# zhuker/lamejs

Hardware: NVIDIA H100
Metric: encoded audio seconds/sec (44.1kHz stereo 128kbps CBR) (higher is better)
Workload: dtype f64

## Files before the change

lamejs_b200/csrc/k_filterbank.cuh:

```cuda
#ifndef MP3B200_K_FILTERBANK_CUH
#define MP3B200_K_FILTERBANK_CUH
#include "mp3_device.cuh"

#define FB_G 8
#define FB_SPAN (576 * FB_G + 1055)
#define FB_PCM_WORDS (FB_SPAN + (FB_SPAN >> 5) + 2)
#define FB_SLAB_STRIDE 33
#define FB_THREADS 192

__constant__ double c_enwindow[285];
__constant__ double c_mdct_win[4 * 36];
__constant__ int c_sb_order[32];

#define EW(i) c_enwindow[(i)]
#define MWIN(t, i) c_mdct_win[(t) * 36 + (i)]
#define WS(i) c_mdct_win[2 * 36 + (i)]
#define SQRT2_D 1.41421356237309504880

__device__ __forceinline__ int fb_pad(int i) { return i + (i >> 5); }

__device__ __forceinline__ void window_subband_dev(const double* __restrict__ x, int p0, f32s* a) {
#define X1(o) (x[fb_pad(x1p + (o))])
#define X2(o) (x[fb_pad(x2p + (o))])
  int x1p = p0, x2p = p0 + 238 - 14 - 286;
// ... 299 lines not shown
  for (int w = tid; w < scount * 18; w += FB_THREADS) {
    const int s = w / 18, j = w - s * 18;
    f32s a[32];
    window_subband_dev(pcm, 576 * s + 286 + 32 * j, a);
    f32s* row = slab + (s * 18 + j) * FB_SLAB_STRIDE;
#pragma unroll
    for (int p = 0; p < 32; p++) {
      double v = a[p];
      if ((j & 1) && (p & 1)) v = v * -1;
      const float amp = s_amp[p];
      f32s r; r = v;
      if ((double)amp < 1.0 && !((double)amp < 1e-12)) r *= (double)amp;
      row[p] = r;
    }
  }
  __syncthreads();
  float* const dst = slab_out + (((size_t)sd.unit_base + z + u0 + 1) * nch + ch) * 576;
  for (int w = tid; w < scount * 576; w += FB_THREADS) {
    const int s = w / 576, r = w - s * 576;
    dst[(size_t)s * nch * 576 + r] = slab[(s * 18 + (r >> 5)) * FB_SLAB_STRIDE + (r & 31)].v;
  }
}

__global__ void __launch_bounds__(FB_G * 32)
k_mdct(const Mp3Tables* __restrict__ T, const StreamDesc* __restrict__ streams, const float* __restrict__ slab_in,
       const signed char* __restrict__ blocktype, float* __restrict__ xr_out) {
  const int z = blockIdx.z;
  const StreamDesc& sd = streams[z];
  const int ch = blockIdx.y;
  const int ngr = sd.nframes * T->mode_gr;
  const int g0 = blockIdx.x * FB_G;
  if (g0 >= ngr) return;
  const int gcount = min(FB_G, ngr - g0);
  const int nch = T->nch;
  __shared__ f32s xr[FB_G * 576];
  __shared__ float s_amp[32];
  __shared__ int s_bt[FB_G];
  const int tid = threadIdx.x;
  if (tid < 32) s_amp[c_sb_order[tid]] = T->amp_filter[tid];
  if (tid < gcount) s_bt[tid] = blocktype[(size_t)(sd.unit_base + g0 + tid) * 2 + ch];
  __syncthreads();

  {
    const int g = tid >> 5, band = tid & 31;
    if (g < gcount) {
      const int type = s_bt[g];
      const int ob = c_sb_order[band];
      f32s* o = xr + g * 576 + band * 18;
      if ((double)s_amp[ob] < 1e-12) {
#pragma unroll
        for (int k = 0; k < 18; k++) o[k] = 0.0;
      } else {
        const float* p0 = slab_in + (((size_t)sd.unit_base + z + g0 + g) * nch + ch) * 576 + ob;
        const float* p1 = p0 + (size_t)nch * 576;
        float b0[18], b1[18];
#pragma unroll
        for (int k = 0; k < 18; k++) { b0[k] = __ldg(p0 + 32 * k); b1[k] = __ldg(p1 + 32 * k); }
#define B0(k) ((double)b0[(k)])
#define B1(k) ((double)b1[(k)])
        if (type == BT_SHORT) {
          f32s io[18];
#pragma unroll
          for (int k = -3; k < 0; k++) {
            const double wv = WS(k + 3);
            io[k * 3 + 9] = B0(9 + k) * wv - B0(8 - k);
            io[k * 3 + 18] = B0(14 - k) * wv + B0(15 + k);
            io[k * 3 + 10] = B0(15 + k) * wv - B0(14 - k);
            io[k * 3 + 19] = B1(2 - k) * wv + B1(3 + k);
            io[k * 3 + 11] = B1(3 + k) * wv - B1(2 - k);
            io[k * 3 + 20] = B1(8 - k) * wv + B1(9 + k);
          }
          mdct_short_dev(io);
#pragma unroll
          for (int k = 0; k < 18; k++) o[k] = (double)io[k];
        } else {
          f32s work[18];
#pragma unroll
          for (int k = -9; k < 0; k++) {
            double a, b;
            a = MWIN(type, k + 27) * B1(k + 9) + MWIN(type, k + 36) * B1(8 - k);
            b = MWIN(type, k + 9) * B0(k + 9) - MWIN(type, k + 18) * B0(8 - k);
            work[k + 9] = a - b * WS(3 + k + 9);
            work[k + 18] = a * WS(3 + k + 9) + b;
          }
          mdct_long_dev(o, work);
        }
#undef B0
#undef B1
      }
    }
  }
  __syncthreads();

  for (int w = tid; w < gcount * 31 * 8; w += FB_G * 32) {
    const int g = w / 248, r = w - g * 248;
    const int band = 1 + (r >> 3), k = r & 7;
    if (s_bt[g] == BT_SHORT) continue;
    f32s* e = xr + g * 576 + band * 18;
    const double lo_v = e[-1 - k], hi_v = e[k];
    const double bu = hi_v * WS(20 + k) + lo_v * WS(28 + k);
    const double bd = hi_v * WS(28 + k) - lo_v * WS(20 + k);
    e[-1 - k] = bu;
    e[k] = bd;
  }
  __syncthreads();
  for (int w = tid; w < gcount * 576; w += FB_G * 32) {
    const int g = w / 576, i = w - g * 576;
    xr_out[((size_t)(sd.unit_base + g0 + g) * nch + ch) * 576 + i] = xr[w].v;
  }
}

#endif
```

lamejs_b200/csrc/k_psy.cuh:

```cuda
#ifndef MP3B200_K_PSY_CUH
#define MP3B200_K_PSY_CUH
#include "mp3_device.cuh"
#include "mp3_tables.h"

#ifndef PSY_THREADS
#define PSY_THREADS 128
#endif
#define MASK_THREADS 128

struct PsyUnit {
  float eb_l[MP3_CBANDS];
  float peaks[9];
  float loudness;
  unsigned char mask_idx[MP3_CBANDS];
  unsigned char attack[4];
  unsigned char pad_;
};
struct PsyShort {
  double ecb_s[3][MP3_CBANDS];
  float eb_s[3][MP3_CBANDS];
};
struct PsyRatioDev { float en_l[22], thm_l[22], en_s[13][3], thm_s[13][3]; };

__constant__ unsigned char c_fft_rv[128];
// ... 683 lines not shown
      return m1 * ((c_table1[i] - f) * r + f);
    }
    if (i > 13) return m1;
    return m1 * c_table3[i];
  }
  return m1 * c_table1[i];
}

__global__ void __launch_bounds__(MASK_THREADS)
k_psy_masking(const Mp3Tables* __restrict__ T, const StreamDesc* __restrict__ streams, const PsyUnit* __restrict__ psy,
              const PsyShort* __restrict__ psy_s, const signed char* __restrict__ bt_prev, const signed char* __restrict__ bt_final,
              int all_short, const double* __restrict__ ath_psy, PsyRatioDev* __restrict__ ratio) {
  const int z = blockIdx.z;
  const StreamDesc& sd = streams[z];
  const int u = (int)blockIdx.x - 1;
  if (u >= T->mode_gr * sd.nframes) return;
  const int nch = T->nch;
  const long long c = (long long)T->mode_gr * sd.frame0 + u;
  const int tid = threadIdx.x, ch = tid >> 6, b = tid & 63;
  PsyRatioDev* out = ratio + psy_row(sd, z, u) * nch;
  if (u < 0) {
    if (c < 0) {
      const float big = (float)1e20;
      for (int i = tid; i < nch * 122; i += MASK_THREADS) (&out[0].en_l[0])[i] = big;
    }
    else if (sd.halo_in) {
      for (int i = tid; i < nch * 122; i += MASK_THREADS) (&out[0].en_l[0])[i] = sd.halo_in[i];
    }
    return;
  }
  __shared__ f32s s_thr[2][MP3_CBANDS + 2], s_eb[2][MP3_CBANDS + 2];
  __shared__ f32s s_thr_s[2][3][MP3_CBANDS + 2];
  __shared__ PsyRatioDev s_out[2];
  const int npl = T->npart_l, nps = T->npart_s;
  const PsyUnit* pu = (ch < nch) ? psy + psy_row(sd, z, u) * nch + ch : nullptr;
  const PsyShort* ps = (ch < nch) ? psy_s + psy_row(sd, z, u) * nch + ch : nullptr;
  const PsyShort* pp = (ch < nch) ? psy_s + psy_row(sd, z, u - 1) * nch + ch : nullptr;
  const bool short_read = psy_short_read(T, sd, bt_final, u, all_short);
  const double ath_adjust = ath_psy[sd.frame_base + u / T->mode_gr];

  if (ch < nch) {
    if (b < npl) {
      int kk = T->s3lo_l[b];
      int k = T->s3off_l[b];
      double eb2 = (double)pu->eb_l[kk] * c_tab[pu->mask_idx[kk]];
      double ecb = (double)T->s3_ll[k++] * eb2;
      while (++kk <= T->s3hi_l[b]) {
        eb2 = (double)pu->eb_l[kk] * c_tab[pu->mask_idx[kk]];
        ecb = mask_add_dev(ecb, (double)T->s3_ll[k++] * eb2, kk, kk - b, T, ath_adjust);
      }
// ... 59 lines not shown
      if (bd >= 0) {
        const double w_curr = (double)T->bo_s_weight[sbi];
        en[sbi][sblock] += w_curr * (double)ps->eb_s[sblock][bd];
        thm[sbi][sblock] += w_curr * (double)s_thr_s[ch][sblock][bd];
      }
    }
    const double e3 = (double)pu->peaks[sblock * 3 + 0], e4 = (double)pu->peaks[sblock * 3 + 1], e5 = (double)pu->peaks[sblock * 3 + 2];
    double t = (double)thm[sbi][sblock];
    t *= 0.8;
    const double enn2 = e3 + e4 + e5;
    if (e5 * 6 < enn2) { t *= 0.5; if (e4 * 6 < enn2) t *= 0.5; }
    thm[sbi][sblock] = t;
  }
  __syncthreads();
  if (nch == 2 && T->interch_ratio > 0.0 && tid < (short_read ? 22 + 39 : 22)) {
    const double r = T->interch_ratio;
    f32s* t0 = reinterpret_cast<f32s*>(tid < 22 ? &s_out[0].thm_l[tid] : &s_out[0].thm_s[0][0] + (tid - 22));
    f32s* t1 = reinterpret_cast<f32s*>(tid < 22 ? &s_out[1].thm_l[tid] : &s_out[1].thm_s[0][0] + (tid - 22));
    const double l = (double)*t0, rr = (double)*t1;
    *t0 += rr * r;
    *t1 += l * r;
  }
  __syncthreads();
  for (int i = tid; i < nch * 122; i += MASK_THREADS)
    if (short_read || i % 122 < 44) (&out[0].en_l[0])[i] = (&s_out[0].en_l[0])[i];
  if (sd.halo_out && u == T->mode_gr * sd.nframes - 1)
    for (int i = tid; i < nch * 122; i += MASK_THREADS) sd.halo_out[i] = (&s_out[0].en_l[0])[i];
}

#endif
```

lamejs_b200/csrc/k_quant.cuh:

```cuda
#ifndef MP3B200_K_QUANT_CUH
#define MP3B200_K_QUANT_CUH
#include <stddef.h>
#include "mp3_device.cuh"
#include "mp3_tables.h"
#include "k_psy.cuh"

#define Q_LARGE_BITS 100000
#define Q_IXMAX 8206
#define Q_FULL 0xffffffffu

struct GranuleInfoDev {
  int global_gain, part2_3_length, part2_length, big_values, count1, scalefac_compress;
  int table_select[3], region0_count, region1_count, preflag, scalefac_scale, count1table_select, block_type;
  int subblock_gain[4];
  int count1bits, sfbmax, sfbdivide, sfb_lmax, psymax, psy_lmax, sfb_smin, max_nonzero_coeff;
  int scalefac[MP3_SFBMAX];
  int slen[4];
  int part_row;
  int pad_;
  double xrpow_max;
};
struct QuantFrameState {
  int stream, rel_frame;
  int in_old[2], in_step[2];
// ... 829 lines not shown
    } else {
      if (++age > search_limit && best.over_count == 0) break;
    }
    const int cont = (wk->w.global_gain + wk->w.scalefac_scale) < 255;
    __syncwarp();
    if (!cont) break;
  } while (true);
  if (!best_here) copy_ix_w(wk->ixw, wk->ixg);
}

__device__ __noinline__ double ath_adjust_dev(double a, double x, double athFloor) {
  const double o = 90.30873362, p = 94.82444863;
  double u = q_log10(x) * 10.0;
  const double v = a * a;
  double w = 0.0;
  u -= athFloor;
  if (v > 1E-20) w = 1. + q_log10(v) * (10.0 / o);
  if (w < 0) w = 0.;
  u *= w;
  u += athFloor + o - p;
  return q_pow(10., 0.1 * u);
}

__device__ __noinline__ bool gc_prepare_w(const Mp3Tables* T, GcWork* wk, const double* ath_ps, const float* __restrict__ xr_g, int block_type,
                             const PsyRatioDev* __restrict__ ratio, double ath_adjust) {
  const bool need_xmin = true;
  const int lane = LANE;
  GranuleInfoDev* gi = &wk->b;
  const bool is_short = block_type == BT_SHORT;
  if (lane == 0) {
    gi->part2_3_length = 0; gi->big_values = 0; gi->count1 = 0; gi->global_gain = 210; gi->scalefac_compress = 0;
    gi->table_select[0] = gi->table_select[1] = gi->table_select[2] = 0;
    gi->subblock_gain[0] = gi->subblock_gain[1] = gi->subblock_gain[2] = gi->subblock_gain[3] = 0;
    gi->region0_count = 0; gi->region1_count = 0; gi->preflag = 0; gi->scalefac_scale = 0; gi->count1table_select = 0;
    gi->part2_length = 0; gi->block_type = block_type; gi->count1bits = 0;
    gi->sfb_lmax = is_short ? 0 : 21; gi->sfb_smin = is_short ? 0 : 12;
    gi->psy_lmax = is_short ? 0 : 21;
    gi->psymax = is_short ? 36 : 21; gi->sfbmax = is_short ? 36 : 21; gi->sfbdivide = is_short ? 18 : 11;
    gi->max_nonzero_coeff = 575;
#pragma unroll 1
    for (int i = 0; i < MP3_SFBMAX; i++) gi->scalefac[i] = 0;
    gi->xrpow_max = 0;
  }
  const Mp3Geo* geo = &T->geo[is_short ? 1 : 0];
  if (lane == 0) wk->geo = geo;
  {
    float4 v[5];
#pragma unroll
    for (int k = 0; k < 5; k++) { const int q = lane + 32 * k; if (q < 144) v[k] = __ldg(reinterpret_cast<const float4*>(xr_g) + q); }
    if (!is_short) {
#pragma unroll
      for (int k = 0; k < 5; k++) { const int q = lane + 32 * k; if (q < 144) reinterpret_cast<float4*>(wk->xr)[q] = v[k]; }
    } else {
#pragma unroll
      for (int k = 0; k < 5; k++) {
        const int q = lane + 32 * k;
        if (q < 144) {
          const short* ro = geo->reorder + 4 * q;
          wk->xr[__ldg(ro + 0)] = v[k].x; wk->xr[__ldg(ro + 1)] = v[k].y; wk->xr[__ldg(ro + 2)] = v[k].z; wk->xr[__ldg(ro + 3)] = v[k].w;
        }
      }
    }
  }
  __syncwarp();
  if (!is_short) {
    const int lo = T->psfb21[0];
    const double lf = (double)T->longfact[21];
    int keep = lo - 1;
#pragma unroll 1
    for (int j = lo + lane; j < 576; j += 32) {
      int g = 0;
      while (g < 5 && j >= T->psfb21[g + 1]) g++;
      double ath21 = ath_ps[g];
      if (lf > 1e-12) ath21 *= lf;
      if (!(fabs((double)wk->xr[j]) < ath21)) keep = j;
    }
    keep = wmax(keep);
    __syncwarp();
#pragma unroll 1
    for (int j = keep + 1 + lane; j < 576; j += 32) wk->xr[j] = 0.0f;
  } else if (lane == 0) {
#pragma unroll 1
    for (int block = 0; block < 3; block++) {
      bool stop = false;
#pragma unroll 1
// ... 585 lines not shown

__device__ __forceinline__ int granule_budget(int nch, int mean_bits, int gr, int used0, int used1, int ch) {
  int tbits = mean_bits;
  if (gr == 1) {
    const int resv = -(used0 + (nch == 2 ? used1 : 0)) + mean_bits;
    if (resv * 10 > 0) tbits += resv;
  }
  double t = (double)tbits / nch;
  if (t > 4095) t = 4095;
  int targ = (int)t;
  const int bits = targ * nch;
  if (bits > 7680) { targ = targ * 7680; targ = (int)((double)targ / bits); }
  (void)ch;
  return targ;
}

#ifndef Q_WARPS
#define Q_WARPS 4
#endif
#ifndef Q_BLOCKS_PER_SM
#define Q_BLOCKS_PER_SM 7
#endif
#define Q_THREADS (32 * Q_WARPS)

__device__ __forceinline__ int next_task(int* counter) {
  int t = 0;
  if (LANE == 0) t = atomicAdd(counter, 1);
  return __shfl_sync(Q_FULL, t, 0);
}
template <int STRIDE = (int)sizeof(WarpShared)>
__device__ __forceinline__ WarpShared* warp_shared() {
  extern __shared__ __align__(16) unsigned char smem_raw[];
  return reinterpret_cast<WarpShared*>(smem_raw + (threadIdx.x >> 5) * STRIDE);
}
__device__ __forceinline__ void gi_init_w(GranuleInfoDev* gi, const GcPrep* __restrict__ pr) {
  __syncwarp();
  int* w = reinterpret_cast<int*>(gi);
#pragma unroll 1
  for (int i = LANE; i < (int)(sizeof(GranuleInfoDev) / 4); i += 32) w[i] = 0;
  __syncwarp();
  if (LANE == 0) {
    const int bt = pr->block_type;
    const bool is_short = bt == BT_SHORT;
    gi->global_gain = 210; gi->block_type = bt;
    gi->sfb_lmax = is_short ? 0 : 21; gi->sfb_smin = is_short ? 0 : 12; gi->psy_lmax = is_short ? 0 : 21;
    gi->psymax = is_short ? 36 : 21; gi->sfbmax = is_short ? 36 : 21; gi->sfbdivide = is_short ? 18 : 11;
// ... 2 lines not shown
  __syncwarp();
}
__device__ __forceinline__ void copy_row16_w(void* dst, const void* src, int nbytes) {
  __syncwarp();
  const int n = nbytes >> 4;
  int4 v[5];
#pragma unroll
  for (int k = 0; k < 5; k++) { const int i = LANE + 32 * k; if (i < n) v[k] = reinterpret_cast<const int4*>(src)[i]; }
#pragma unroll
  for (int k = 0; k < 5; k++) { const int i = LANE + 32 * k; if (i < n) reinterpret_cast<int4*>(dst)[i] = v[k]; }
  __syncwarp();
}
struct FrameGeom { int z, f, padding, frame_bytes, mean_bits; long long kabs; };
__device__ __forceinline__ FrameGeom frame_geom(const Mp3Tables* T, const StreamDesc* streams, const QuantFrameState* q) {
  FrameGeom g;
  g.z = q->stream; g.f = q->rel_frame;
  g.kabs = (long long)streams[g.z].frame0 + g.f;
  g.padding = (int)(pad_count(g.kabs, T->frac_SpF, T->samplerate) - pad_count(g.kabs - 1, T->frac_SpF, T->samplerate));
  g.frame_bytes = T->frame_bytes_nopad + g.padding;
  g.mean_bits = (8 * g.frame_bytes - T->sideinfo_len * 8) / T->mode_gr;
  return g;
}

__global__ void __launch_bounds__(Q_THREADS, Q_BLOCKS_PER_SM)
k_q_prepare(const Mp3Tables* __restrict__ T, const StreamDesc* __restrict__ streams, const float* __restrict__ xr,
            const PsyRatioDev* __restrict__ ratio, const signed char* __restrict__ bt_final, const double* __restrict__ ath_q,
            const QuantFrameState* __restrict__ qs, float* __restrict__ xrq, float* __restrict__ xrpow_g, unsigned* __restrict__ neg_g,
            GcPrep* __restrict__ prep,
            int nframes, int* __restrict__ counter) {
  WarpShared* ws = warp_shared();
  GcWork* wk = &ws->wk;
  const int lane = LANE, nch = T->nch;
  const int G = T->mode_gr;
  const int ntasks = nframes * G * nch;
#pragma unroll 1
  for (int t = next_task(counter); t < ntasks; t = next_task(counter)) {
    const int frow = t / (G * nch), rem = t - frow * G * nch, gr = rem / nch, ch = rem - gr * nch;
    const QuantFrameState* q = qs + frow;
    const int z = q->stream, f = q->rel_frame;
    const StreamDesc& sd = streams[z];
    const double ath_adjust = ath_q[frow];
    const size_t urow = (size_t)sd.unit_base + G * f + gr, gidx = urow * nch + ch;
    const int bt = bt_final[urow * 2 + ch];
    const PsyRatioDev* rt = ratio + ((size_t)sd.unit_base + z + G * f + gr) * nch + ch;
    __syncwarp();
    if (lane < 6) ws->ath[lane] = ath_adjust_dev(ath_adjust, (double)(bt == BT_SHORT ? T->ath_psfb12[lane] : T->ath_psfb21[lane]), T->ath_floor);
    __syncwarp();
    const bool have = gc_prepare_w(T, wk, ws->ath, xr + gidx * 576, bt, rt, ath_adjust);
    copy_row16_w(xrq + gidx * 576, wk->xr, 2304);
    {
      unsigned mine = 0;
#pragma unroll 1
      for (int k = 0; k < 18; k++) { const unsigned m = __ballot_sync(Q_FULL, wk->xr[lane + 32 * k] < 0.0f); if (lane == k) mine = m; }
      if (lane < 18) neg_g[gidx * 18 + lane] = mine;
    }
    copy_row16_w(xrpow_g + gidx * 576, wk->xrpow, 2304);
    GcPrep* pr = prep + gidx;
#pragma unroll 1
    for (int i = lane; i < MP3_SFBMAX; i += 32) pr->xmin[i] = wk->xmin[i];
    if (lane == 0) { pr->have = have ? 1 : 0; pr->mnz = wk->b.max_nonzero_coeff; pr->block_type = bt; pr->xrpow_max = wk->b.xrpow_max; }
  }
}

__global__ void __launch_bounds__(Q_THREADS, Q_SLIM_BLOCKS)
k_q_search(const Mp3Tables* __restrict__ T, const StreamDesc* __restrict__ streams, QuantFrameState* __restrict__ qs,
           GranuleInfoDev* __restrict__ ginfo, short* __restrict__ l3enc, const float* __restrict__ xrpow_g,
           const GcPrep* __restrict__ prep, int gr, const int* __restrict__ list, const int* __restrict__ count_ptr, int count_direct,
           int revalidate, int* __restrict__ counter, int* __restrict__ list2, int* __restrict__ count2,
           int* __restrict__ list3, int* __restrict__ count3) {
  WarpShared* ws = warp_shared<Q_STRIDE_NOXR>();
  GcWork* wk = &ws->wk;
// ... 260 lines not shown

__global__ void k_qstate_commit(StreamDesc* __restrict__ streams, int nstreams, const QuantFrameState* __restrict__ qs) {
  const int z = blockIdx.x * blockDim.x + threadIdx.x;
  if (z >= nstreams) return;
  StreamDesc& sd = streams[z];
  if (sd.nframes <= 0) return;
  const QuantFrameState* q = qs + sd.frame_base + sd.nframes - 1;
#pragma unroll 1
  for (int c = 0; c < 2; c++) { sd.old_value[c] = q->out_old[c]; sd.current_step[c] = q->out_step[c]; }
}

__global__ void k_qstate_loop_cond(cudaGraphConditionalHandle loop, int* __restrict__ count, int* __restrict__ st, int max_passes) {
  const int n = *count;
  int passes = st[2];
  bool more = n != 0;
  if (more) passes++;
  if (passes > max_passes) { st[1] = 1; *count = 0; more = false; }
  st[2] = passes;
  if (passes > st[0]) st[0] = passes;
  cudaGraphSetConditional(loop, more ? 1u : 0u);
}

struct QuantBuffers {
  const float* xr; const PsyRatioDev* ratio; const signed char* bt; const double* ath_q;
  QuantFrameState* qs; GranuleInfoDev* ginfo; short* l3enc; float* xrq; float* xrpow; unsigned* neg; GcPrep* prep;
  int* over_budget;
  int* list; int* counter;
};
#define Q_NCOUNTERS 256
#define Q_REPAIR_BLOCKS 16
enum { QE_START, QE_PREP, QE_S0, QE_O0, QE_F0, QE_S1, QE_MID, QE_O1, QE_F1, QE_PK, QE_COUNT };

struct QuantLoop {
  cudaStream_t capture = nullptr;
  int* st = nullptr;
  cudaGraphExec_t exec = nullptr;
};

static int quant_run(const Mp3Tables* dT, const Mp3Tables& hT, StreamDesc* d_streams, int S, int nstreams_with_frames, int max_frames, long long F,
                     const QuantBuffers& B, cudaStream_t st_main, cudaStream_t st_repair, cudaEvent_t ev_fork, cudaEvent_t ev_join,
                     cudaEvent_t ev_pass1, cudaEvent_t* evq, int* evq_pred, int* passes_out, std::atomic<long long>* launches,
                     QuantLoop* dloop = nullptr) {
  cudaStream_t st = st_main;
  static std::mutex attr_mu;
  static bool attr_done[64] = {};
  int dev = 0, sms = 132;
  cudaGetDevice(&dev);
// ... 12 lines not shown
  }
  if (F <= 0) { *passes_out = 0; return 0; }
  const int nch = hT.nch;
  int next_counter = Q_NCOUNTERS;
  auto fresh_counter = [&]() -> int* {
    if (next_counter >= Q_NCOUNTERS) { cudaMemsetAsync(B.counter + 3, 0, sizeof(int) * (Q_NCOUNTERS - 3), st); next_counter = 3; }
    return B.counter + next_counter++;
  };
  auto grid_for = [&](long long tasks, int per_sm) -> int {
    long long g = (tasks + Q_WARPS - 1) / Q_WARPS, cap = (long long)sms * per_sm;
    if (g > cap) g = cap;
    return (int)(g < 1 ? 1 : g);
  };
  {
    dim3 g((max_frames + 127) / 128, S);
    k_qstate_init<<<g, 128, 0, st>>>(d_streams, S, B.qs);
    (*launches)++;
  }
  for (int i = 0; i < QE_COUNT; i++) evq_pred[i] = -1;
  int last_slot = -1;
  auto mark = [&](int slot) { cudaEventRecord(evq[slot], st); evq_pred[slot] = last_slot; last_slot = slot; };
  int* const prep_counter = fresh_counter();
  mark(QE_START);
  k_q_prepare<<<grid_for(F * hT.mode_gr * nch, Q_BLOCKS_PER_SM), Q_THREADS, smem, st>>>(dT, d_streams, B.xr, B.ratio, B.bt, B.ath_q, B.qs, B.xrq, B.xrpow, B.neg,
                                                                              B.prep, (int)F, prep_counter);
  mark(QE_PREP);
  (*launches)++;
  int* const list1 = B.list;
  int* const list2 = B.list + (F + 1);
  int* const list3 = B.list + 2 * (F + 1);
  auto search = [&](int gr, const int* list, const int* cptr, long long count, int reval) {
    k_q_search<<<grid_for(count * nch, Q_SLIM_BLOCKS), Q_THREADS, smem_slim, st>>>(dT, d_streams, B.qs, B.ginfo, B.l3enc, B.xrpow, B.prep, gr, list, cptr, (int)count,
                                                                             reval, fresh_counter(), list2, B.counter + 1, list3, B.counter + 2);
    (*launches)++;
  };
  int reserve_blocks = 0;
  auto finish = [&](int gr, const int* list, const int* cptr, long long count, int reval) {
    k_q_finish<<<max(1, grid_for(count * nch, Q_SLIM_BLOCKS) - reserve_blocks), Q_THREADS, smem_slim, st>>>(dT, d_streams, B.qs, B.ginfo, B.l3enc, gr, list, cptr, (int)count, reval, fresh_counter());
    (*launches)++;
  };
  auto outer = [&](int gr, const int* list, const int* cptr, long long count, int reval) {
    k_q_outer<<<max(1, grid_for(count * nch, Q_BLOCKS_PER_SM) - reserve_blocks), Q_THREADS, smem, st>>>(dT, d_streams, B.qs, B.ginfo, B.l3enc, B.xrq, B.xrpow, B.prep, gr, list, cptr, (int)count,
                                                                            reval, fresh_counter());
    (*launches)++;
  };
  auto outer_finish = [&](int gr, long long count, int reval, int slot_o, int slot_f) {
    outer(gr, nullptr, nullptr, count, reval); mark(slot_o);
    finish(gr, nullptr, nullptr, count, reval); mark(slot_f);
  };
  auto pack = [&](const int* list, const int* cptr, long long count, int reval) {
// ... 117 lines not shown
```

lamejs_b200/csrc/mp3_encoder.cu:

```cuda
#include <cuda_runtime.h>
#include <math.h>
#include <stdio.h>
#include <algorithm>
#include <array>
#include <stdlib.h>
#include <string.h>
#include <atomic>
#include <map>
#include <mutex>
#include <string>
#include <tuple>
#include <vector>

#include "../../include/mp3b200.h"
#include "mp3_config.h"
#include "mp3_device.cuh"
#include "mp3_tables.h"
#include "k_filterbank.cuh"
#include "k_psy.cuh"
#include "k_quant.cuh"
#include "k_tag.cuh"
#include "k_resample.cuh"
#include "k_replaygain.cuh"
#include "k_stage.cuh"
// ... 164 lines not shown
  Buf<int> short_count;
  Buf<ScanIn> scan_in;
  Buf<PsyRatioDev> ratio;
  Buf<double> ath_psy;
  Buf<double> ath_q;
  Buf<QuantFrameState> qstate;
  Buf<GranuleInfoDev> ginfo;
  Buf<short> l3enc;
  Buf<float> xrq;
  Buf<float> xrpow;
  Buf<unsigned> neg;
  Buf<GcPrep> prep;
  Buf<int> dirty;
  Buf<int> counter;
  Buf<ScanChunk> scan;
  Buf<ResampleDesc> rs_desc;
  Buf<float> rs_y;
  Buf<StageDesc> st_desc;
  Buf<float> st_y;
  Buf<int> refusals;
  int fit(int S, int nch, long long U, long long F) {
    const size_t gc = (size_t)U * nch, rows = (size_t)(U + S) * nch, f = (size_t)F + 1;
    const bool failed = streams.fit(S) || bt_final.fit((size_t)U * 2 + 16) || bt_prev.fit((size_t)U * 2 + 16) ||
                        xr.fit(gc * 576) || slab.fit(rows * 576) || psy.fit(rows) || psy_s.fit(rows) || short_list.fit(rows) ||
                        short_count.fit(2) || scan_in.fit(rows) || ratio.fit(rows) ||
                        ath_psy.fit(f) || ath_q.fit(f) || qstate.fit(f) || ginfo.fit(gc) || l3enc.fit(gc * 576) ||
                        xrq.fit(gc * 576) || xrpow.fit(gc * 576) || neg.fit(gc * 18) || prep.fit(gc) || dirty.fit(3 * f) ||
                        counter.fit(Q_NCOUNTERS) || scan.fit((size_t)(F / SCAN_FRAMES + S + 1));
    return failed ? MP3B200_ERR_CUDA : 0;
  }
  size_t generation() const {
    return streams.cap + qstate.cap + ginfo.cap + l3enc.cap + xrq.cap + xrpow.cap + neg.cap + prep.cap + dirty.cap + counter.cap +
           refusals.cap;
  }
  void release() {
    streams.release(); bt_final.release(); bt_prev.release(); xr.release(); slab.release(); psy.release(); psy_s.release(); short_list.release();
    short_count.release(); scan_in.release();
    ratio.release(); ath_psy.release(); ath_q.release(); qstate.release(); ginfo.release(); l3enc.release(); xrq.release();
    xrpow.release(); neg.release(); prep.release(); dirty.release(); counter.release(); scan.release();
    rs_desc.release(); rs_y.release(); st_desc.release(); st_y.release(); refusals.release();
  }
};

struct PinnedArena { uint8_t* p = nullptr; size_t cap = 0, used = 0; };

enum { MP3_MAX_PCM_CHUNKS = 8 };
enum { MP3_MAX_LAUNCH_STREAMS = 65535 };
// ... 130 lines not shown

struct Timings { float psy = 0, scan = 0, mask = 0, fb = 0, q1 = 0, qn = 0, total = 0; int passes = 0;
                 float q_prepare = 0, q_search = 0, q_outer = 0, q_finish = 0, q_pack = 0, q_mid = 0; };

struct PcmArrival { int chunks = 1; cudaEvent_t* ready = nullptr; };

int refusal_error(int refused, int over_budget, int fault) {
  if (refused) { g_err = "non-finite input sample (or one beyond 2^40 once scaled)"; return MP3B200_ERR_CONFIG; }
  if (over_budget) { g_err = "frame over its bit budget (input too loud to encode)"; return MP3B200_ERR_CONFIG; }
  if (fault == RG_FAULT) { g_err = "ReplayGain repair did not converge"; return MP3B200_ERR_CUDA; }
  if (fault) { g_err = "quantizer stage failed: the fixed-point loop did not converge"; return MP3B200_ERR_CUDA; }
  return 0;
}

int check_refusals(ThreadCtx& c) {
  int r[2] = {0, 0};
  CK(cudaMemcpyAsync(r, c.ws.refusals.p, sizeof r, cudaMemcpyDeviceToHost, c.st));
  CK(cudaStreamSynchronize(c.st));
  return refusal_error(r[0], r[1], 0);
}

struct LaunchOpts {
  const int32_t* force_bt = nullptr;
  bool stop_after_mdct = false;
  bool all_short = false;
  const PcmArrival* arrival = nullptr;
  float* timings_ms = nullptr;
  bool sync = true;
  struct RgJob* rg = nullptr;
  bool f32_in = false;
  struct LoopGraphs* loops = nullptr;
  const struct HandleCarry* carry = nullptr;
  int* rg_loop = nullptr;
  bool analyse_only = false;
};

struct HandleCarry { HandleRecord* const* recs; float* halo_scratch; };

enum { MP3_RG_GRAPHS = 32 };
struct LoopGraphs {
  cudaStream_t capture = nullptr;
  size_t generation = 0, rg_generation = 0;
  long long instantiated = 0;
  unsigned long long rg_tick = 0;
  std::map<std::tuple<const Config*, int, long long, int>, cudaGraphExec_t> exec;
  struct RgGraph { cudaGraphExec_t exec = nullptr; unsigned long long used = 0; };
  std::map<std::tuple<const Config*, bool, int, int, long long, const int*>, RgGraph> rg_exec;
// ... 198 lines not shown
    std::vector<signed char> bt((size_t)units * 2, 0);
    for (long long u = 0; u < units; u++)
      for (int c = 0; c < nch; c++) bt[u * 2 + c] = (signed char)o.force_bt[u * nch + c];
    CK(cudaMemcpyAsync(ws.bt_final.p, bt.data(), bt.size(), cudaMemcpyHostToDevice, st));
    CK(cudaStreamSynchronize(st));
  }
  {
    CK(cudaMemsetAsync(ws.short_count.p, 0, 2 * sizeof(int), st));
    dim3 grid((cfg->host.mode_gr * max_frames + 1 + 127) / 128, S);
    k_psy_short_list<<<grid, 128, 0, st>>>(tab, ws.streams.p, ws.bt_final.p, o.all_short ? 1 : 0, ws.short_list.p, ws.short_count.p);
    DBG("k_psy_short_list");
    int sms = 132;
    CK(cudaDeviceGetAttribute(&sms, cudaDevAttrMultiProcessorCount, c.device));
    const long long tasks = ((long long)cfg->host.mode_gr * total_frames + S) * nch;
    const int blocks = (int)std::min<long long>(std::max<long long>(tasks, 1), (long long)sms * PSY_SHORT_BLOCKS);
    if (f32_pcm) k_psy_short<true><<<blocks, PSY_THREADS, 0, st>>>(tab, ws.streams.p, ws.psy_s.p, ws.short_list.p, ws.short_count.p);
    else k_psy_short<false><<<blocks, PSY_THREADS, 0, st>>>(tab, ws.streams.p, ws.psy_s.p, ws.short_list.p, ws.short_count.p);
    g_launches += 2;
    DBG("k_psy_short");
    if (psy_launch >= 0 && (rc = psy_record_short(c, h_streams, nch, cfg->host.mode_gr, psy_launch, k2_launches))) return rc;
  }
  {
    dim3 grid(cfg->host.mode_gr * max_frames + 1, 1, S);
    k_psy_masking<<<grid, MASK_THREADS, 0, st>>>(tab, ws.streams.p, ws.psy.p, ws.psy_s.p, ws.bt_prev.p, ws.bt_final.p,
                                                 o.all_short ? 1 : 0, ws.ath_psy.p, ws.ratio.p);
    g_launches++;
    DBG("k_psy_masking");
  }
  CK(cudaEventRecord(ev[3], st));
  {
    dim3 grid((cfg->host.mode_gr * max_frames + FB_G - 1) / FB_G, nch, S);
    k_mdct<<<grid, FB_G * 32, 0, st>>>(tab, ws.streams.p, ws.slab.p, ws.bt_final.p, ws.xr.p);
    g_launches++;
    DBG("k_mdct");
  }
  CK(cudaEventRecord(ev[4], st));
  int passes = 0;
  if (!o.stop_after_mdct) {
    QuantBuffers qb;
    qb.xr = ws.xr.p; qb.ratio = ws.ratio.p; qb.bt = ws.bt_final.p; qb.ath_q = ws.ath_q.p; qb.qs = ws.qstate.p; qb.ginfo = ws.ginfo.p;
    qb.l3enc = ws.l3enc.p; qb.xrq = ws.xrq.p; qb.xrpow = ws.xrpow.p; qb.neg = ws.neg.p; qb.prep = ws.prep.p; qb.list = ws.dirty.p; qb.counter = ws.counter.p;
    qb.over_budget = ws.refusals.p + 1;
    QuantLoop dloop;
    cudaGraphExec_t* cached = nullptr;
    if (o.loops) {
      LoopGraphs& lg = *o.loops;
      if (lg.generation != ws.generation()) { lg.clear(); lg.generation = ws.generation(); }
      cached = &lg.exec[std::make_tuple((const Config*)cfg, S, total_frames, max_frames)];
      dloop.capture = lg.capture; dloop.st = ws.refusals.p + 2; dloop.exec = *cached;
    }
    rc = quant_run(tab, cfg->host, ws.streams.p, S, streams_with_frames, max_frames, total_frames, qb, st, c.aux_st, c.ev_fork, c.ev_join, ev[5], c.evq, c.evq_pred, &passes, &g_launches,
                   o.loops ? &dloop : nullptr);
    if (cached) {
      if (!*cached && dloop.exec) o.loops->instantiated++;
      *cached = dloop.exec;
      if (!dloop.exec) o.loops->exec.erase(std::make_tuple((const Config*)cfg, S, total_frames, max_frames));
    }
    if (rc) { g_err = "quantizer stage failed: " + std::string(cudaGetErrorString(cudaGetLastError())); return rc; }
  } else {
    CK(cudaEventRecord(ev[5], st));
  }
  CK(cudaEventRecord(ev[6], st));
  if (!o.sync) return 0;
  CK(cudaStreamSynchronize(st));
  CK(cudaGetLastError());
  if (tm) {
    cudaEventElapsedTime(&tm->psy, ev[0], ev[1]);
    cudaEventElapsedTime(&tm->scan, ev[1], ev[2]);
    cudaEventElapsedTime(&tm->mask, ev[2], ev[3]);
    cudaEventElapsedTime(&tm->fb, ev[3], ev[4]);
    cudaEventElapsedTime(&tm->q1, ev[4], ev[5]);
    cudaEventElapsedTime(&tm->qn, ev[5], ev[6]);
    cudaEventElapsedTime(&tm->total, ev[0], ev[6]);
    tm->passes = passes;
    if (!o.stop_after_mdct && passes > 0) {
      auto span = [&](int slot) { float v = 0; const int p = c.evq_pred[slot]; if (p >= 0) cudaEventElapsedTime(&v, c.evq[p], c.evq[slot]); return v; };
      tm->q_prepare = span(QE_PREP);
      tm->q_search = span(QE_S0) + span(QE_S1);
      tm->q_outer = span(QE_O0) + span(QE_O1);
      tm->q_finish = span(QE_F0) + span(QE_F1);
      tm->q_pack = span(QE_PK);
      tm->q_mid = span(QE_MID);
    }
  }
  return 0;
}

void init_stream_state(StreamDesc& sd) {
  sd.ath_adjust = 0.01; sd.ath_adjust_limit = 1.0;
  sd.blocktype_old[0] = sd.blocktype_old[1] = BT_NORM;
  sd.last_attacks[0] = sd.last_attacks[1] = 0;
  sd.old_value[0] = sd.old_value[1] = 180;
  sd.current_step[0] = sd.current_step[1] = 4;
}

long long hist_base_at(int mode_gr, long long frame) {
  const long long b = 576LL * mode_gr * frame - 1104;
  return b > 0 ? b : 0;
// ... 371 lines not shown
    }
    if (o.rg) {
      rc = rg_queue(c, cfg, group, *o.rg, arrival, rows);
      if (rc) return rc;
    }
    Timings tm;
    rc = o.analyse_only ? 0 : run_pipeline(c, cfg, group, n, o, arrival, rows, &tm);
    if (rc) return rc;
    if (o.rg) {
      rc = o.loops ? rg_finish_queued(c, cfg, *o.rg, *o.loops, o.rg_loop ? o.rg_loop : c.ws.refusals.p + 5, c.ws.refusals.p + 3)
                   : rg_finish(c, cfg, *o.rg);
      if (rc) return rc;
    }
    arrival = nullptr;
    float rs_ms = 0.0f;
    if (resampled && o.timings_ms && o.sync) CK(cudaEventElapsedTime(&rs_ms, c.ev_rs[0], c.ev_rs[1]));
    if (o.timings_ms) {
      const float t[16] = {tm.psy, tm.scan, tm.mask, tm.fb, tm.q1, tm.qn, tm.total, 0.0f,
                           tm.q_prepare, tm.q_search, tm.q_outer, tm.q_finish, tm.q_pack, tm.q_mid, rs_ms, 0.0f};
      for (int i = 0; i < 16; i++) o.timings_ms[i] += t[i];
      if ((float)tm.passes > o.timings_ms[7]) o.timings_ms[7] = (float)tm.passes;
    }
  }
  return o.sync && (o.f32_in || !o.stop_after_mdct) ? check_refusals(c) : 0;
}

}

extern "C" {

const char* mp3b200_last_error(void) { return g_err.c_str(); }
#ifdef Q_STATS
int mp3b200_debug_qstats(unsigned long long* out16, int reset) {
  if (cudaMemcpyFromSymbol(out16, g_qstats, sizeof(unsigned long long) * 16) != cudaSuccess) return MP3B200_ERR_CUDA;
  if (reset) { unsigned long long z[16] = {0}; cudaMemcpyToSymbol(g_qstats, z, sizeof z); }
  return 0;
}
#endif
int64_t mp3b200_launch_count(void) { return g_launches; }
int mp3b200_debug_psy_capture(int on) {
  std::lock_guard<std::mutex> lk(g_psy_mu);
  if (on) { g_psy_rec.clear(); g_psy_launch = 0; }
  g_psy_capture.store(on ? 1 : 0);
  return 0;
}
int64_t mp3b200_debug_psy_take(void* buf, int64_t cap) {
  std::lock_guard<std::mutex> lk(g_psy_mu);
// ... 513 lines not shown
  uint8_t* bytes_out = tp->bytes_out;
  const int64_t bytes_cap = tp->bytes_cap;
  Config* cfg;
  int rc = get_config(channels, tp->samplerate, tp->kbps, tp->flags & ~MP3B200_DEBUG_SKIP_SHORT, &cfg);
  if (rc || (rc = check_input(cfg, 1, &left, &right, &nsamples))) return rc;
  const int nch = cfg->host.nch;
  const int G = cfg->host.mode_gr;
  const StreamPlan pl = stream_plan(cfg, 1, &nsamples, false, nullptr);
  const long long F = pl.frames[0], U = G * F, nbytes = pl.audio[0];
  std::vector<int64_t> pcm_off;
  T* d_pcm = nullptr;
  PcmArrival arr;
  if ((rc = upload_host_rows(cfg, 1, &left, &right, &nsamples, pcm_off, d_pcm, arr)) || (rc = t_ctx.out.fit((size_t)nbytes + 8))) return rc;
  uint8_t* d_out = t_ctx.out.p;
  const int64_t zero = 0;
  std::vector<StreamDesc> sds = whole_streams(cfg, pl, 1, d_pcm, pcm_off.data(), &nsamples, d_out, &zero);
  const bool want_gi = ginfo || tp->scalefac || tp->subblock_gain;
  const bool want_prep = tp->xmin || tp->max_nonzero_coeff || tp->xrpow_max;
  const bool want_q = tp->scfsi || tp->old_value || tp->cur_step;
  LaunchOpts opts;
  opts.f32_in = std::is_same_v<T, float>;
  opts.force_bt = force_blocktype;
  opts.all_short = !(tp->flags & MP3B200_DEBUG_SKIP_SHORT);
  opts.stop_after_mdct = !(l3_enc || bytes_out || want_gi || want_prep || want_q);
  opts.arrival = &arr;
  rc = launch_streams(t_ctx, cfg, sds, opts);
  auto fetch = [](void* dst, const void* src, size_t bytes) {
    const cudaError_t e = cudaMemcpyAsync(dst, src, bytes, cudaMemcpyDeviceToHost, t_ctx.st);
    return e != cudaSuccess ? e : cudaStreamSynchronize(t_ctx.st);
  };
  const Workspace& ws = t_ctx.ws;
  if (rc == 0) {
    if (xr) CK(fetch(xr, ws.xr.p, sizeof(float) * (size_t)U * nch * 576));
    if (blocktype) {
      std::vector<signed char> bt((size_t)U * 2);
      CK(fetch(bt.data(), ws.bt_final.p, bt.size()));
      for (long long u = 0; u < U; u++) for (int c = 0; c < nch; c++) blocktype[u * nch + c] = bt[u * 2 + c];
    }
    if (en_l || thm_l || en_s || thm_s) {
      std::vector<PsyRatioDev> r((size_t)(U + 1) * nch);
      CK(fetch(r.data(), ws.ratio.p, sizeof(PsyRatioDev) * r.size()));
      for (long long u = 0; u < U; u++) for (int c = 0; c < nch; c++) {
        const PsyRatioDev& q = r[(size_t)u * nch + c];
        if (en_l) memcpy(en_l + (u * nch + c) * 22, q.en_l, sizeof q.en_l);
        if (thm_l) memcpy(thm_l + (u * nch + c) * 22, q.thm_l, sizeof q.thm_l);
        if (en_s) memcpy(en_s + (u * nch + c) * 39, q.en_s, sizeof q.en_s);
        if (thm_s) memcpy(thm_s + (u * nch + c) * 39, q.thm_s, sizeof q.thm_s);
// ... 250 lines not shown
```

Measured before the change: 61490.

## Fuse MDCT into quantizer prepare kernel and size masking block by channels

Removes the standalone k_mdct kernel and computes each granule's MDCT, including alias reduction, inside k_q_prepare. One warp does this per granule and writes straight into the working buffer, so the xr round-trip through global memory and one kernel launch go away. The xr buffer is kept only as an optional debug tap, and short-block reordering now happens in shared memory. k_psy_masking is also launched with 64*nch threads, and its strided loops use blockDim, so stereo runs at the same 128 threads. The cost is that MDCT now runs warp-serial per granule inside a kernel tuned for quantizer occupancy, which may add pressure on registers or time.

```diff
diff --git a/lamejs_b200/csrc/k_filterbank.cuh b/lamejs_b200/csrc/k_filterbank.cuh
--- a/lamejs_b200/csrc/k_filterbank.cuh
+++ b/lamejs_b200/csrc/k_filterbank.cuh
@@ -345,92 +345,69 @@
   }
 }
 
-__global__ void __launch_bounds__(FB_G * 32)
-k_mdct(const Mp3Tables* __restrict__ T, const StreamDesc* __restrict__ streams, const float* __restrict__ slab_in,
-       const signed char* __restrict__ blocktype, float* __restrict__ xr_out) {
-  const int z = blockIdx.z;
-  const StreamDesc& sd = streams[z];
-  const int ch = blockIdx.y;
-  const int ngr = sd.nframes * T->mode_gr;
-  const int g0 = blockIdx.x * FB_G;
-  if (g0 >= ngr) return;
-  const int gcount = min(FB_G, ngr - g0);
-  const int nch = T->nch;
-  __shared__ f32s xr[FB_G * 576];
-  __shared__ float s_amp[32];
-  __shared__ int s_bt[FB_G];
-  const int tid = threadIdx.x;
-  if (tid < 32) s_amp[c_sb_order[tid]] = T->amp_filter[tid];
-  if (tid < gcount) s_bt[tid] = blocktype[(size_t)(sd.unit_base + g0 + tid) * 2 + ch];
-  __syncthreads();
-
-  {
-    const int g = tid >> 5, band = tid & 31;
-    if (g < gcount) {
-      const int type = s_bt[g];
-      const int ob = c_sb_order[band];
-      f32s* o = xr + g * 576 + band * 18;
-      if ((double)s_amp[ob] < 1e-12) {
-#pragma unroll
-        for (int k = 0; k < 18; k++) o[k] = 0.0;
-      } else {
-        const float* p0 = slab_in + (((size_t)sd.unit_base + z + g0 + g) * nch + ch) * 576 + ob;
-        const float* p1 = p0 + (size_t)nch * 576;
-        float b0[18], b1[18];
-#pragma unroll
-        for (int k = 0; k < 18; k++) { b0[k] = __ldg(p0 + 32 * k); b1[k] = __ldg(p1 + 32 * k); }
+__device__ __forceinline__ void mdct_granule_w(const Mp3Tables* __restrict__ T, const float* __restrict__ slab_prev, int nch, int type,
+                                               f32s* xr) {
+  const int band = threadIdx.x & 31;
+  {
+    const int ob = c_sb_order[band];
+    f32s* o = xr + band * 18;
+    if ((double)T->amp_filter[band] < 1e-12) {
+#pragma unroll
+      for (int k = 0; k < 18; k++) o[k] = 0.0;
+    } else {
+      const float* p0 = slab_prev + ob;
+      const float* p1 = p0 + (size_t)nch * 576;
+      float b0[18], b1[18];
+#pragma unroll
+      for (int k = 0; k < 18; k++) { b0[k] = __ldg(p0 + 32 * k); b1[k] = __ldg(p1 + 32 * k); }
 #define B0(k) ((double)b0[(k)])
 #define B1(k) ((double)b1[(k)])
-        if (type == BT_SHORT) {
-          f32s io[18];
-#pragma unroll
-          for (int k = -3; k < 0; k++) {
-            const double wv = WS(k + 3);
-            io[k * 3 + 9] = B0(9 + k) * wv - B0(8 - k);
-            io[k * 3 + 18] = B0(14 - k) * wv + B0(15 + k);
-            io[k * 3 + 10] = B0(15 + k) * wv - B0(14 - k);
-            io[k * 3 + 19] = B1(2 - k) * wv + B1(3 + k);
-            io[k * 3 + 11] = B1(3 + k) * wv - B1(2 - k);
-            io[k * 3 + 20] = B1(8 - k) * wv + B1(9 + k);
-          }
-          mdct_short_dev(io);
-#pragma unroll
-          for (int k = 0; k < 18; k++) o[k] = (double)io[k];
-        } else {
-          f32s work[18];
-#pragma unroll
-          for (int k = -9; k < 0; k++) {
-            double a, b;
-            a = MWIN(type, k + 27) * B1(k + 9) + MWIN(type, k + 36) * B1(8 - k);
-            b = MWIN(type, k + 9) * B0(k + 9) - MWIN(type, k + 18) * B0(8 - k);
-            work[k + 9] = a - b * WS(3 + k + 9);
-            work[k + 18] = a * WS(3 + k + 9) + b;
-          }
-          mdct_long_dev(o, work);
+      if (type == BT_SHORT) {
+        f32s io[18];
+#pragma unroll
+        for (int k = -3; k < 0; k++) {
+          const double wv = WS(k + 3);
+          io[k * 3 + 9] = B0(9 + k) * wv - B0(8 - k);
+          io[k * 3 + 18] = B0(14 - k) * wv + B0(15 + k);
+          io[k * 3 + 10] = B0(15 + k) * wv - B0(14 - k);
+          io[k * 3 + 19] = B1(2 - k) * wv + B1(3 + k);
+          io[k * 3 + 11] = B1(3 + k) * wv - B1(2 - k);
+          io[k * 3 + 20] = B1(8 - k) * wv + B1(9 + k);
         }
+        mdct_short_dev(io);
+#pragma unroll
+        for (int k = 0; k < 18; k++) o[k] = (double)io[k];
+      } else {
+        f32s work[18];
+#pragma unroll
+        for (int k = -9; k < 0; k++) {
+          double a, b;
+          a = MWIN(type, k + 27) * B1(k + 9) + MWIN(type, k + 36) * B1(8 - k);
+          b = MWIN(type, k + 9) * B0(k + 9) - MWIN(type, k + 18) * B0(8 - k);
+          work[k + 9] = a - b * WS(3 + k + 9);
+          work[k + 18] = a * WS(3 + k + 9) + b;
+        }
+        mdct_long_dev(o, work);
+      }
 #undef B0
 #undef B1
-      }
     }
   }
-  __syncthreads();
-
-  for (int w = tid; w < gcount * 31 * 8; w += FB_G * 32) {
-    const int g = w / 248, r = w - g * 248;
-    const int band = 1 + (r >> 3), k = r & 7;
-    if (s_bt[g] == BT_SHORT) continue;
-    f32s* e = xr + g * 576 + band * 18;
-    const double lo_v = e[-1 - k], hi_v = e[k];
-    const double bu = hi_v * WS(20 + k) + lo_v * WS(28 + k);
-    const double bd = hi_v * WS(28 + k) - lo_v * WS(20 + k);
-    e[-1 - k] = bu;
-    e[k] = bd;
-  }
-  __syncthreads();
-  for (int w = tid; w < gcount * 576; w += FB_G * 32) {
-    const int g = w / 576, i = w - g * 576;
-    xr_out[((size_t)(sd.unit_base + g0 + g) * nch + ch) * 576 + i] = xr[w].v;
-  }
+  __syncwarp();
+
+  if (type != BT_SHORT) {
+#pragma unroll 1
+    for (int r = band; r < 31 * 8; r += 32) {
+      f32s* e = xr + (1 + (r >> 3)) * 18;
+      const int k = r & 7;
+      const double lo_v = e[-1 - k], hi_v = e[k];
+      const double bu = hi_v * WS(20 + k) + lo_v * WS(28 + k);
+      const double bd = hi_v * WS(28 + k) - lo_v * WS(20 + k);
+      e[-1 - k] = bu;
+      e[k] = bd;
+    }
+  }
+  __syncwarp();
 }
 
 #endif
diff --git a/lamejs_b200/csrc/k_psy.cuh b/lamejs_b200/csrc/k_psy.cuh
--- a/lamejs_b200/csrc/k_psy.cuh
+++ b/lamejs_b200/csrc/k_psy.cuh
@@ -729,10 +729,10 @@
   if (u < 0) {
     if (c < 0) {
       const float big = (float)1e20;
-      for (int i = tid; i < nch * 122; i += MASK_THREADS) (&out[0].en_l[0])[i] = big;
+      for (int i = tid; i < nch * 122; i += (int)blockDim.x) (&out[0].en_l[0])[i] = big;
     }
     else if (sd.halo_in) {
-      for (int i = tid; i < nch * 122; i += MASK_THREADS) (&out[0].en_l[0])[i] = sd.halo_in[i];
+      for (int i = tid; i < nch * 122; i += (int)blockDim.x) (&out[0].en_l[0])[i] = sd.halo_in[i];
     }
     return;
   }
@@ -838,10 +838,10 @@
     *t1 += l * r;
   }
   __syncthreads();
-  for (int i = tid; i < nch * 122; i += MASK_THREADS)
+  for (int i = tid; i < nch * 122; i += (int)blockDim.x)
     if (short_read || i % 122 < 44) (&out[0].en_l[0])[i] = (&s_out[0].en_l[0])[i];
   if (sd.halo_out && u == T->mode_gr * sd.nframes - 1)
-    for (int i = tid; i < nch * 122; i += MASK_THREADS) sd.halo_out[i] = (&s_out[0].en_l[0])[i];
-}
-
-#endif
+    for (int i = tid; i < nch * 122; i += (int)blockDim.x) sd.halo_out[i] = (&s_out[0].en_l[0])[i];
+}
+
+#endif
diff --git a/lamejs_b200/csrc/k_quant.cuh b/lamejs_b200/csrc/k_quant.cuh
--- a/lamejs_b200/csrc/k_quant.cuh
+++ b/lamejs_b200/csrc/k_quant.cuh
@@ -875,7 +875,7 @@
   return q_pow(10., 0.1 * u);
 }
 
-__device__ __noinline__ bool gc_prepare_w(const Mp3Tables* T, GcWork* wk, const double* ath_ps, const float* __restrict__ xr_g, int block_type,
+__device__ __noinline__ bool gc_prepare_w(const Mp3Tables* T, GcWork* wk, const double* ath_ps, int block_type,
                              const PsyRatioDev* __restrict__ ratio, double ath_adjust) {
   const bool need_xmin = true;
   const int lane = LANE;
@@ -897,23 +897,13 @@
   }
   const Mp3Geo* geo = &T->geo[is_short ? 1 : 0];
   if (lane == 0) wk->geo = geo;
-  {
-    float4 v[5];
-#pragma unroll
-    for (int k = 0; k < 5; k++) { const int q = lane + 32 * k; if (q < 144) v[k] = __ldg(reinterpret_cast<const float4*>(xr_g) + q); }
-    if (!is_short) {
-#pragma unroll
-      for (int k = 0; k < 5; k++) { const int q = lane + 32 * k; if (q < 144) reinterpret_cast<float4*>(wk->xr)[q] = v[k]; }
-    } else {
-#pragma unroll
-      for (int k = 0; k < 5; k++) {
-        const int q = lane + 32 * k;
-        if (q < 144) {
-          const short* ro = geo->reorder + 4 * q;
-          wk->xr[__ldg(ro + 0)] = v[k].x; wk->xr[__ldg(ro + 1)] = v[k].y; wk->xr[__ldg(ro + 2)] = v[k].z; wk->xr[__ldg(ro + 3)] = v[k].w;
-        }
-      }
-    }
+  if (is_short) {
+    __syncwarp();
+#pragma unroll 1
+    for (int i = lane; i < 576; i += 32) wk->xrpow[i] = wk->xr[i];
+    __syncwarp();
+#pragma unroll 1
+    for (int i = lane; i < 576; i += 32) wk->xr[__ldg(geo->reorder + i)] = wk->xrpow[i];
   }
   __syncwarp();
   if (!is_short) {
@@ -1545,6 +1535,9 @@
 #define Q_BLOCKS_PER_SM 7
 #endif
 #define Q_THREADS (32 * Q_WARPS)
+#ifndef Q_PREP_BLOCKS
+#define Q_PREP_BLOCKS Q_BLOCKS_PER_SM
+#endif
 
 __device__ __forceinline__ int next_task(int* counter) {
   int t = 0;
@@ -1593,9 +1586,9 @@
   return g;
 }
 
-__global__ void __launch_bounds__(Q_THREADS, Q_BLOCKS_PER_SM)
-k_q_prepare(const Mp3Tables* __restrict__ T, const StreamDesc* __restrict__ streams, const float* __restrict__ xr,
-            const PsyRatioDev* __restrict__ ratio, const signed char* __restrict__ bt_final, const double* __restrict__ ath_q,
+__global__ void __launch_bounds__(Q_THREADS, Q_PREP_BLOCKS)
+k_q_prepare(const Mp3Tables* __restrict__ T, const StreamDesc* __restrict__ streams, const float* __restrict__ slab,
+            float* __restrict__ xr_tap, const PsyRatioDev* __restrict__ ratio, const signed char* __restrict__ bt_final, const double* __restrict__ ath_q,
             const QuantFrameState* __restrict__ qs, float* __restrict__ xrq, float* __restrict__ xrpow_g, unsigned* __restrict__ neg_g,
             GcPrep* __restrict__ prep,
             int nframes, int* __restrict__ counter) {
@@ -1615,9 +1608,11 @@
     const int bt = bt_final[urow * 2 + ch];
     const PsyRatioDev* rt = ratio + ((size_t)sd.unit_base + z + G * f + gr) * nch + ch;
     __syncwarp();
+    mdct_granule_w(T, slab + (((size_t)sd.unit_base + z + G * f + gr) * nch + ch) * 576, nch, bt, reinterpret_cast<f32s*>(wk->xr));
+    if (xr_tap) copy_row16_w(xr_tap + gidx * 576, wk->xr, 2304);
     if (lane < 6) ws->ath[lane] = ath_adjust_dev(ath_adjust, (double)(bt == BT_SHORT ? T->ath_psfb12[lane] : T->ath_psfb21[lane]), T->ath_floor);
     __syncwarp();
-    const bool have = gc_prepare_w(T, wk, ws->ath, xr + gidx * 576, bt, rt, ath_adjust);
+    const bool have = gc_prepare_w(T, wk, ws->ath, bt, rt, ath_adjust);
     copy_row16_w(xrq + gidx * 576, wk->xr, 2304);
     {
       unsigned mine = 0;
@@ -1924,7 +1919,10 @@
 }
 
 struct QuantBuffers {
-  const float* xr; const PsyRatioDev* ratio; const signed char* bt; const double* ath_q;
+  const float* slab;
+  float* xr_tap;
+  bool prepare_only;
+  const PsyRatioDev* ratio; const signed char* bt; const double* ath_q;
   QuantFrameState* qs; GranuleInfoDev* ginfo; short* l3enc; float* xrq; float* xrpow; unsigned* neg; GcPrep* prep;
   int* over_budget;
   int* list; int* counter;
@@ -1983,10 +1981,11 @@
   auto mark = [&](int slot) { cudaEventRecord(evq[slot], st); evq_pred[slot] = last_slot; last_slot = slot; };
   int* const prep_counter = fresh_counter();
   mark(QE_START);
-  k_q_prepare<<<grid_for(F * hT.mode_gr * nch, Q_BLOCKS_PER_SM), Q_THREADS, smem, st>>>(dT, d_streams, B.xr, B.ratio, B.bt, B.ath_q, B.qs, B.xrq, B.xrpow, B.neg,
+  k_q_prepare<<<grid_for(F * hT.mode_gr * nch, Q_PREP_BLOCKS), Q_THREADS, smem, st>>>(dT, d_streams, B.slab, B.xr_tap, B.ratio, B.bt, B.ath_q, B.qs, B.xrq, B.xrpow, B.neg,
                                                                               B.prep, (int)F, prep_counter);
   mark(QE_PREP);
   (*launches)++;
+  if (B.prepare_only) { *passes_out = 0; return 0; }
   int* const list1 = B.list;
   int* const list2 = B.list + (F + 1);
   int* const list3 = B.list + 2 * (F + 1);
diff --git a/lamejs_b200/csrc/mp3_encoder.cu b/lamejs_b200/csrc/mp3_encoder.cu
--- a/lamejs_b200/csrc/mp3_encoder.cu
+++ b/lamejs_b200/csrc/mp3_encoder.cu
@@ -210,7 +210,7 @@
   int fit(int S, int nch, long long U, long long F) {
     const size_t gc = (size_t)U * nch, rows = (size_t)(U + S) * nch, f = (size_t)F + 1;
     const bool failed = streams.fit(S) || bt_final.fit((size_t)U * 2 + 16) || bt_prev.fit((size_t)U * 2 + 16) ||
-                        xr.fit(gc * 576) || slab.fit(rows * 576) || psy.fit(rows) || psy_s.fit(rows) || short_list.fit(rows) ||
+                        slab.fit(rows * 576) || psy.fit(rows) || psy_s.fit(rows) || short_list.fit(rows) ||
                         short_count.fit(2) || scan_in.fit(rows) || ratio.fit(rows) ||
                         ath_psy.fit(f) || ath_q.fit(f) || qstate.fit(f) || ginfo.fit(gc) || l3enc.fit(gc * 576) ||
                         xrq.fit(gc * 576) || xrpow.fit(gc * 576) || neg.fit(gc * 18) || prep.fit(gc) || dirty.fit(3 * f) ||
@@ -387,7 +387,8 @@
 
 struct LaunchOpts {
   const int32_t* force_bt = nullptr;
-  bool stop_after_mdct = false;
+  bool stop_after_prepare = false;
+  bool taps = false;
   bool all_short = false;
   const PcmArrival* arrival = nullptr;
   float* timings_ms = nullptr;
@@ -632,23 +633,19 @@
   }
   {
     dim3 grid(cfg->host.mode_gr * max_frames + 1, 1, S);
-    k_psy_masking<<<grid, MASK_THREADS, 0, st>>>(tab, ws.streams.p, ws.psy.p, ws.psy_s.p, ws.bt_prev.p, ws.bt_final.p,
-                                                 o.all_short ? 1 : 0, ws.ath_psy.p, ws.ratio.p);
+    k_psy_masking<<<grid, 64 * nch, 0, st>>>(tab, ws.streams.p, ws.psy.p, ws.psy_s.p, ws.bt_prev.p, ws.bt_final.p,
+                                             o.all_short ? 1 : 0, ws.ath_psy.p, ws.ratio.p);
     g_launches++;
     DBG("k_psy_masking");
   }
   CK(cudaEventRecord(ev[3], st));
-  {
-    dim3 grid((cfg->host.mode_gr * max_frames + FB_G - 1) / FB_G, nch, S);
-    k_mdct<<<grid, FB_G * 32, 0, st>>>(tab, ws.streams.p, ws.slab.p, ws.bt_final.p, ws.xr.p);
-    g_launches++;
-    DBG("k_mdct");
-  }
   CK(cudaEventRecord(ev[4], st));
   int passes = 0;
-  if (!o.stop_after_mdct) {
+  {
+    if (o.taps && ws.xr.fit((size_t)cfg->host.mode_gr * total_frames * nch * 576)) return MP3B200_ERR_CUDA;
     QuantBuffers qb;
-    qb.xr = ws.xr.p; qb.ratio = ws.ratio.p; qb.bt = ws.bt_final.p; qb.ath_q = ws.ath_q.p; qb.qs = ws.qstate.p; qb.ginfo = ws.ginfo.p;
+    qb.slab = ws.slab.p; qb.xr_tap = o.taps ? ws.xr.p : nullptr; qb.prepare_only = o.stop_after_prepare;
+    qb.ratio = ws.ratio.p; qb.bt = ws.bt_final.p; qb.ath_q = ws.ath_q.p; qb.qs = ws.qstate.p; qb.ginfo = ws.ginfo.p;
     qb.l3enc = ws.l3enc.p; qb.xrq = ws.xrq.p; qb.xrpow = ws.xrpow.p; qb.neg = ws.neg.p; qb.prep = ws.prep.p; qb.list = ws.dirty.p; qb.counter = ws.counter.p;
     qb.over_budget = ws.refusals.p + 1;
     QuantLoop dloop;
@@ -667,8 +664,7 @@
       if (!dloop.exec) o.loops->exec.erase(std::make_tuple((const Config*)cfg, S, total_frames, max_frames));
     }
     if (rc) { g_err = "quantizer stage failed: " + std::string(cudaGetErrorString(cudaGetLastError())); return rc; }
-  } else {
-    CK(cudaEventRecord(ev[5], st));
+    if (o.stop_after_prepare) CK(cudaEventRecord(ev[5], st));
   }
   CK(cudaEventRecord(ev[6], st));
   if (!o.sync) return 0;
@@ -683,7 +679,7 @@
     cudaEventElapsedTime(&tm->qn, ev[5], ev[6]);
     cudaEventElapsedTime(&tm->total, ev[0], ev[6]);
     tm->passes = passes;
-    if (!o.stop_after_mdct && passes > 0) {
+    if (!o.stop_after_prepare && passes > 0) {
       auto span = [&](int slot) { float v = 0; const int p = c.evq_pred[slot]; if (p >= 0) cudaEventElapsedTime(&v, c.evq[p], c.evq[slot]); return v; };
       tm->q_prepare = span(QE_PREP);
       tm->q_search = span(QE_S0) + span(QE_S1);
@@ -1101,7 +1097,7 @@
       if ((float)tm.passes > o.timings_ms[7]) o.timings_ms[7] = (float)tm.passes;
     }
   }
-  return o.sync && (o.f32_in || !o.stop_after_mdct) ? check_refusals(c) : 0;
+  return o.sync && (o.f32_in || !o.stop_after_prepare) ? check_refusals(c) : 0;
 }
 
 }
@@ -1661,7 +1657,8 @@
   opts.f32_in = std::is_same_v<T, float>;
   opts.force_bt = force_blocktype;
   opts.all_short = !(tp->flags & MP3B200_DEBUG_SKIP_SHORT);
-  opts.stop_after_mdct = !(l3_enc || bytes_out || want_gi || want_prep || want_q);
+  opts.stop_after_prepare = !(l3_enc || bytes_out || want_gi || want_prep || want_q);
+  opts.taps = xr != nullptr;
   opts.arrival = &arr;
   rc = launch_streams(t_ctx, cfg, sds, opts);
   auto fetch = [](void* dst, const void* src, size_t bytes) {
```

Result: faster. 63030, median of 6 (+2.5%).
